# nirschl-lab/stain2stain

Measured on AMD Instinct MI355X. Metric: paired 256x256 stain tiles/sec (full CFM optimisation step), higher is better.
Workload: dtype bf16

## Files before the change

stain2stain_amd/csrc/conv3x3_wgrad_mfma.hip:

```cpp
#include "common.h"
#include <stdlib.h>
#include <type_traits>

struct WgradArgs {
  const void* dy;
  const void* x0;
  const void* x1;
  float* part;
  int lddy, Cout, ld0, c0, ld1, c1;
  int B, H, W, tilesY, tilesX, ntiles, S;
  int lgc;
  int lgh, lgw;
  int xcd;
};

namespace {

template <typename T> struct WPiece;
template <> struct WPiece<bf16_t> {
  bf16x8 v;
  __device__ __forceinline__ void zero() {
#pragma unroll
    for (int i = 0; i < 8; ++i) v[i] = (bf16_t)0.0f;
  }
  __device__ __forceinline__ void load(const bf16_t* p) { v = *reinterpret_cast<const bf16x8*>(p); }
  __device__ __forceinline__ void to_lds(char* hi, int, int off) const { *reinterpret_cast<bf16x8*>(hi + off) = v; }
};
template <> struct WPiece<float> {
  f32x4 a, b;
  __device__ __forceinline__ void zero() {
#pragma unroll
    for (int i = 0; i < 4; ++i) { a[i] = 0.f; b[i] = 0.f; }
  }
  __device__ __forceinline__ void load(const float* p) {
    a = *reinterpret_cast<const f32x4*>(p);
    b = *reinterpret_cast<const f32x4*>(p + 4);
  }
  __device__ __forceinline__ void to_lds(char* hi, int img_stride, int off) const {
    bf16x8 h, m, l;
#pragma unroll
    for (int i = 0; i < 8; ++i) {
      const float x = i < 4 ? a[i] : b[i - 4];
      h[i] = (bf16_t)x;
      const float r1 = x - (float)h[i];
      m[i] = (bf16_t)r1;
      l[i] = (bf16_t)(r1 - (float)m[i]);
    }
    *reinterpret_cast<bf16x8*>(hi + off) = h;
    *reinterpret_cast<bf16x8*>(hi + img_stride + off) = m;
    *reinterpret_cast<bf16x8*>(hi + 2 * img_stride + off) = l;
  }
};

typedef __attribute__((address_space(3))) s16x4 lds_s16x4;

__device__ __forceinline__ bf16x8 tr_frag(const char* p_rows0, int row_stride4) {
  s16x4 lo = __builtin_amdgcn_ds_read_tr16_b64_v4i16((lds_s16x4*)(p_rows0));
  s16x4 hi = __builtin_amdgcn_ds_read_tr16_b64_v4i16((lds_s16x4*)(p_rows0 + row_stride4));
  bf16x4 l4 = __builtin_bit_cast(bf16x4, lo), h4 = __builtin_bit_cast(bf16x4, hi);
  bf16x8 r;
#pragma unroll
  for (int i = 0; i < 4; ++i) { r[i] = l4[i]; r[4 + i] = h4[i]; }
  return r;
}

template <typename T, int TH, int TW>
__global__ __launch_bounds__(256, (std::is_same<T, float>::value ? 1 : 2)) void conv3x3_wgrad_kernel(WgradArgs a) {
  constexpr bool SPLIT = std::is_same<T, float>::value;
  constexpr int NIMG = SPLIT ? 3 : 1;
  constexpr int NPX = TH * TW;
  constexpr int HW_ = TW + 2, HALO = (TH + 2) * HW_;
  constexpr int DY_BYTES = 2 * NPX * 64;
  constexpr int X_BYTES = 2 * HALO * 64;
  constexpr int DY_PIECES = NPX * 8, DY_IT = (DY_PIECES + 255) / 256;
  constexpr int X_PIECES = HALO * 8, X_IT = (X_PIECES + 255) / 256;
  constexpr int KSTEPS = NPX / 16;
  static_assert(TW % 16 == 0, "a k-step is 16 consecutive pixels of one tile row");

  extern __shared__ __attribute__((aligned(16))) char smem[];
  char* const ldsDY = smem;
  char* const ldsX = smem + NIMG * DY_BYTES;

  const T* __restrict__ dy = static_cast<const T*>(a.dy);
  const T* __restrict__ x0 = static_cast<const T*>(a.x0);
  const T* __restrict__ x1 = static_cast<const T*>(a.x1);

  const int tid = threadIdx.x, lane = tid & 63, wave = tid >> 6;
  const int wco = wave >> 1, wci = wave & 1;
  const int ci0 = blockIdx.x * 64, co0 = blockIdx.y * 64;
  const int cin = a.c0 + a.c1;

  const int g = lane >> 4, q = (lane & 15) >> 2, p = lane & 3;
  const int frag_off = ((g >> 1) * 8 + q) * 64 + ((g & 1) * 16 + p * 4) * 2;

  f32x16 acc[9];
#pragma unroll
  for (int t = 0; t < 9; ++t)
#pragma unroll
    for (int j = 0; j < 16; ++j) acc[t][j] = 0.f;

  WPiece<T> dreg[DY_IT];
  WPiece<T> xreg[X_IT];

  auto load_tile = [&](int tile) {
    int bt = tile;
    const int tx = bt % a.tilesX; bt /= a.tilesX;
    const int ty = bt % a.tilesY;
    const int img = bt / a.tilesY;
    const int y0 = ty * TH, xs = tx * TW;
#pragma unroll
    for (int i = 0; i < DY_IT; ++i) {
      const int idx = tid + i * 256;
      const int px = idx >> 3, pc = idx & 7;
      const int py = px / TW, pxx = px - py * TW;
      const int gy = y0 + py, gx = xs + pxx, co = co0 + pc * 8;
      dreg[i].zero();
      if (idx < DY_PIECES && gy < a.H && gx < a.W && co < a.Cout)
        dreg[i].load(dy + ((long)(img * a.H + gy) * a.W + gx) * a.lddy + co);
    }
#pragma unroll
    for (int i = 0; i < X_IT; ++i) {
      const int idx = tid + i * 256;
      const int px = idx >> 3, pc = idx & 7;
      const int hy = px / HW_, hx = px - hy * HW_;
      const int gy = y0 - 1 + hy, gx = xs - 1 + hx, ci = ci0 + pc * 8;
      xreg[i].zero();
      if (idx < X_PIECES && gy >= 0 && gy < a.H && gx >= 0 && gx < a.W) {
        const long pix = (long)(img * a.H + gy) * a.W + gx;
        if (ci < a.c0) xreg[i].load(x0 + pix * a.ld0 + ci);
        else if (ci < cin) xreg[i].load(x1 + pix * a.ld1 + (ci - a.c0));
      }
    }
  };
  auto store_tile = [&]() {
#pragma unroll
    for (int i = 0; i < DY_IT; ++i) {
      const int idx = tid + i * 256;
      const int px = idx >> 3, pc = idx & 7;
      if (idx < DY_PIECES)
        dreg[i].to_lds(ldsDY, DY_BYTES, (pc >> 2) * (NPX * 64) + px * 64 + (pc & 3) * 16);
    }
#pragma unroll
    for (int i = 0; i < X_IT; ++i) {
      const int idx = tid + i * 256;
      const int px = idx >> 3, pc = idx & 7;
      if (idx < X_PIECES)
        xreg[i].to_lds(ldsX, X_BYTES, (pc >> 2) * (HALO * 64) + px * 64 + (pc & 3) * 16);
    }
  };

  const char* const Ahi = ldsDY + wco * (NPX * 64) + frag_off;
  const char* const Bhi = ldsX + wci * (HALO * 64) + frag_off;

  int tile = blockIdx.z;
  if (tile < a.ntiles) load_tile(tile);
  for (; tile < a.ntiles; tile += a.S) {
    __syncthreads();
    store_tile();
    __syncthreads();
    if (tile + a.S < a.ntiles) load_tile(tile + a.S);
#pragma unroll
    for (int ks = 0; ks < KSTEPS; ++ks) {
      const int m0 = ks * 16;
      const int py = m0 / TW, px = m0 - py * TW;
      const bf16x8 af = tr_frag(Ahi + m0 * 64, 4 * 64);
      bf16x8 am, al;
// ... 3 lines not shown
      }
#pragma unroll
      for (int tap = 0; tap < 9; ++tap) {
        const int hoff = ((py + tap / 3) * HW_ + px + tap % 3) * 64;
        const bf16x8 bfr = tr_frag(Bhi + hoff, 4 * 64);
        if constexpr (SPLIT) {
          const bf16x8 bm = tr_frag(Bhi + X_BYTES + hoff, 4 * 64);
          const bf16x8 bl = tr_frag(Bhi + 2 * X_BYTES + hoff, 4 * 64);
          acc[tap] = __builtin_amdgcn_mfma_f32_32x32x16_bf16(am, bm, acc[tap], 0, 0, 0);
          acc[tap] = __builtin_amdgcn_mfma_f32_32x32x16_bf16(al, bfr, acc[tap], 0, 0, 0);
          acc[tap] = __builtin_amdgcn_mfma_f32_32x32x16_bf16(af, bl, acc[tap], 0, 0, 0);
          acc[tap] = __builtin_amdgcn_mfma_f32_32x32x16_bf16(am, bfr, acc[tap], 0, 0, 0);
          acc[tap] = __builtin_amdgcn_mfma_f32_32x32x16_bf16(af, bm, acc[tap], 0, 0, 0);
        }
        acc[tap] = __builtin_amdgcn_mfma_f32_32x32x16_bf16(af, bfr, acc[tap], 0, 0, 0);
      }
    }
  }

  const int r = lane & 31, h = lane >> 5;
  const int ci = ci0 + wci * 32 + r;
#pragma unroll
  for (int tap = 0; tap < 9; ++tap) {
#pragma unroll
    for (int j = 0; j < 16; ++j) {
      const int co = co0 + wco * 32 + (j & 3) + 8 * (j >> 2) + 4 * h;
      if (co < a.Cout && ci < cin)
        a.part[(((long)blockIdx.z * 9 + tap) * a.Cout + co) * cin + ci] = acc[tap][j];
    }
  }
}

__device__ __attribute__((aligned(64))) char g_wgrad_zero_page[64];
typedef __attribute__((address_space(3))) void lds_void_t;
typedef __attribute__((address_space(1))) const void gbl_void_t;

__device__ __forceinline__ void dma16_asm(const void* gsrc, unsigned lds_dst) {
  unsigned keep;
  asm volatile("s_mov_b32 %0, m0\n\ts_mov_b32 m0, %2\n\ts_nop 0\n\tglobal_load_lds_dwordx4 %1, off\n\ts_mov_b32 m0, %0"
               : "=&s"(keep) : "v"(gsrc), "s"(lds_dst) : "memory");
}

template <int TH, int TW>
__global__ __launch_bounds__(256, 2) void conv3x3_wgrad_dma_kernel(WgradArgs a) {
  using T = bf16_t;
  constexpr int NW = 4, NT = 9;
  constexpr int NPX = TH * TW;
  constexpr int HW_ = TW + 2, HR = TH + 2, HALO = HR * HW_;
  constexpr int XROWS = (HALO + 31) / 32 * 32;
  constexpr int DY_BYTES = 2 * NPX * 64, X_BYTES = 2 * XROWS * 64;
  constexpr int DYGRP = 2 * NPX / 16, XGRP = 2 * XROWS / 16;
  constexpr int DYG = DYGRP / NW;
  constexpr int XG = XGRP / NW;
  constexpr int BUF = DY_BYTES + X_BYTES;
  constexpr int KSTEPS = NPX / 16;
  static_assert(DYGRP % 4 == 0 && XGRP % 4 == 0, "DMA groups split evenly over 4 waves");

  extern __shared__ __attribute__((aligned(16))) char smem[];
  const T* __restrict__ dy = static_cast<const T*>(a.dy);
  const T* __restrict__ x0 = static_cast<const T*>(a.x0);
  const T* __restrict__ x1 = static_cast<const T*>(a.x1);

  const int tid = threadIdx.x, lane = tid & 63;
  const int wave = __builtin_amdgcn_readfirstlane(tid >> 6);
  const int wco = (wave & 3) >> 1, wci = wave & 1;
  unsigned bx = blockIdx.x, by = blockIdx.y, bz = blockIdx.z;
  if (a.xcd) {
    const unsigned L = bx + gridDim.x * (by + gridDim.y * bz), per = gridDim.x * gridDim.y * gridDim.z / 8;
    unsigned Lq = (L & 7) * per + (L >> 3);
    bx = Lq % gridDim.x; Lq /= gridDim.x;
    by = Lq % gridDim.y; bz = Lq / gridDim.y;
  }
  const int ci0 = bx * 64, co0 = by * 64;
  const int cin = a.c0 + a.c1;
  const int drow = lane >> 2, dslot = lane & 3;
  const int zsplit = (int)bz;

  const int g = lane >> 4, q = (lane & 15) >> 2, p = lane & 3;
  const int frag_off = ((g >> 1) * 8 + q) * 64 + ((g & 1) * 16 + p * 4) * 2;

  f32x16 acc[NT];
#pragma unroll
  for (int t = 0; t < NT; ++t)
#pragma unroll
    for (int j = 0; j < 16; ++j) acc[t][j] = 0.f;

  int dy_off[DYG], dy_py[DYG], dy_px[DYG];
  bool dy_ok[DYG];
#pragma unroll
  for (int j = 0; j < DYG; ++j) {
    const int grp = wave + NW * j;
    const int half = grp / (NPX / 16), px = (grp % (NPX / 16)) * 16 + drow;
    const int co = co0 + half * 32 + dslot * 8;
    dy_py[j] = px / TW; dy_px[j] = px - dy_py[j] * TW;
    dy_ok[j] = co < a.Cout;
    dy_off[j] = (dy_py[j] * a.W + dy_px[j]) * a.lddy + co;
  }
  const T* x_ptr[XG];
  int x_off[XG], x_ld[XG], x_hy[XG], x_hx[XG];
#pragma unroll
  for (int j = 0; j < XG; ++j) {
    const int grp = wave + NW * j;
    const int half = grp / (XROWS / 16), px = (grp % (XROWS / 16)) * 16 + drow;
    const int ci = ci0 + half * 32 + dslot * 8;
    x_hy[j] = px / HW_; x_hx[j] = px - x_hy[j] * HW_;
    x_ptr[j] = nullptr; x_ld[j] = 0;
    if (px < HALO) {
      if (ci < a.c0) { x_ptr[j] = x0 + ci; x_ld[j] = a.ld0; }
      else if (ci < cin) { x_ptr[j] = x1 + (ci - a.c0); x_ld[j] = a.ld1; }
    }
    x_off[j] = ((x_hy[j] - 1) * a.W + (x_hx[j] - 1)) * x_ld[j];
  }

  auto dma_tile = [&](int tile, int buf) {
    int bt = tile;
    const int tx = bt % a.tilesX; bt /= a.tilesX;
    const int ty = bt % a.tilesY;
    const int img = bt / a.tilesY;
    const int y0 = ty * TH, xs = tx * TW;
    const long pixbase = (long)(img * a.H + y0) * a.W + xs;
    const bool interior = y0 >= 1 && y0 + TH + 1 <= a.H && xs >= 1 && xs + TW + 1 <= a.W;
    const unsigned base = (unsigned)(uintptr_t)(__attribute__((address_space(3))) char*)smem + buf * BUF;
    if (interior) {
#pragma unroll
      for (int j = 0; j < DYG; ++j) {
        const void* src = dy_ok[j] ? (const void*)(dy + pixbase * a.lddy + dy_off[j]) : (const void*)g_wgrad_zero_page;
        dma16_asm(src, __builtin_amdgcn_readfirstlane(base + (wave + NW * j) * 1024));
      }
#pragma unroll
      for (int j = 0; j < XG; ++j) {
        const void* src = x_ptr[j] ? (const void*)(x_ptr[j] + pixbase * x_ld[j] + x_off[j]) : (const void*)g_wgrad_zero_page;
        dma16_asm(src, __builtin_amdgcn_readfirstlane(base + DY_BYTES + (wave + NW * j) * 1024));
      }
    } else {
#pragma unroll
      for (int j = 0; j < DYG; ++j) {
        const int gy = y0 + dy_py[j], gx = xs + dy_px[j];
        const void* src = g_wgrad_zero_page;
        if (gy < a.H && gx < a.W && dy_ok[j]) src = dy + pixbase * a.lddy + dy_off[j];
        dma16_asm(src, __builtin_amdgcn_readfirstlane(base + (wave + NW * j) * 1024));
      }
#pragma unroll
      for (int j = 0; j < XG; ++j) {
        const int gy = y0 - 1 + x_hy[j], gx = xs - 1 + x_hx[j];
        const void* src = g_wgrad_zero_page;
        if (x_ptr[j] && gy >= 0 && gy < a.H && gx >= 0 && gx < a.W) src = x_ptr[j] + pixbase * x_ld[j] + x_off[j];
        dma16_asm(src, __builtin_amdgcn_readfirstlane(base + DY_BYTES + (wave + NW * j) * 1024));
      }
    }
  };

  int tile = zsplit;
  int buf = 0;
  if (tile < a.ntiles) dma_tile(tile, 0);
  asm volatile("s_waitcnt vmcnt(0)" ::: "memory");
  __builtin_amdgcn_s_barrier();
  for (; tile < a.ntiles; tile += a.S) {
    if (tile + a.S < a.ntiles) dma_tile(tile + a.S, buf ^ 1);
    const char* const Ahi = smem + buf * BUF + wco * (NPX * 64) + frag_off;
    const char* const Bhi = smem + buf * BUF + DY_BYTES + wci * (XROWS * 64) + frag_off;
#pragma unroll
    for (int ks = 0; ks < KSTEPS; ++ks) {
      const int m0 = ks * 16;
      const int py = m0 / TW, px = m0 - py * TW;
      const bf16x8 af = tr_frag(Ahi + m0 * 64, 4 * 64);
#pragma unroll
      for (int t = 0; t < NT; ++t) {
        const int hoff = ((py + t / 3) * HW_ + px + t % 3) * 64;
        const bf16x8 bfr = tr_frag(Bhi + hoff, 4 * 64);
        acc[t] = __builtin_amdgcn_mfma_f32_32x32x16_bf16(af, bfr, acc[t], 0, 0, 0);
      }
    }
    __builtin_amdgcn_sched_barrier(0);
    asm volatile("s_waitcnt vmcnt(0)" ::: "memory");
    __builtin_amdgcn_s_barrier();
    buf ^= 1;
  }

  const int r = lane & 31, h = lane >> 5;
  const int ci = ci0 + wci * 32 + r;
#pragma unroll
  for (int t = 0; t < NT; ++t) {
#pragma unroll
    for (int j = 0; j < 16; ++j) {
      const int co = co0 + wco * 32 + (j & 3) + 8 * (j >> 2) + 4 * h;
      if (co < a.Cout && ci < cin)
        a.part[(((long)zsplit * 9 + t) * a.Cout + co) * cin + ci] = acc[t][j];
    }
  }
}

template <int ZG>
__global__ __launch_bounds__(64 * ZG) void wgrad_reduce_kernel(const float* __restrict__ part, float* __restrict__ grad, int S, int Cout,
                                    int Cin, int accumulate) {
  __shared__ float tile[ZG][9][65];
  const long n = (long)Cout * Cin;
  const int il = threadIdx.x & 63, zg = threadIdx.x >> 6;
  const long i = (long)blockIdx.x * 64 + il;
  float s[9];
#pragma unroll
  for (int t = 0; t < 9; ++t) s[t] = 0.f;
  if (i < n) {
    for (int z = zg; z < S; z += ZG)
#pragma unroll
      for (int t = 0; t < 9; ++t) s[t] += part[((long)z * 9 + t) * n + i];
  }
#pragma unroll
  for (int t = 0; t < 9; ++t) tile[zg][t][il] = s[t];
  __syncthreads();
  const long base = (long)blockIdx.x * 64 * 9;
  for (int k = threadIdx.x; k < 576; k += 64 * ZG) {
    const long o = base + k;
    if (o < n * 9) {
      const int t = k % 9, j = k / 9;
      float v = 0.f;
#pragma unroll
      for (int g = 0; g < ZG; g += 4) v += (tile[g][t][j] + tile[g + 1][t][j]) + (tile[g + 2][t][j] + tile[g + 3][t][j]);
      grad[o] = accumulate ? grad[o] + v : v;
    }
  }
}

template <typename T, int TH, int TW>
int launch_wgrad(WgradArgs& a, hipStream_t s) {
  constexpr int NIMG = std::is_same<T, float>::value ? 3 : 1;
  constexpr int lds = NIMG * (2 * TH * TW * 64 + 2 * (TH + 2) * (TW + 2) * 64);
  a.tilesY = cdiv(a.H, TH);
  a.tilesX = cdiv(a.W, TW);
  a.ntiles = a.B * a.tilesY * a.tilesX;
  if (a.S > a.ntiles) return S2S_ERR_SHAPE;
  auto kern = conv3x3_wgrad_kernel<T, TH, TW>;
  static unsigned long long attr_devs = 0;
  if (int rc = s2s_allow_dyn_lds(reinterpret_cast<const void*>(kern), lds, &attr_devs)) return rc;
  dim3 grid(cdiv(a.c0 + a.c1, 64), cdiv(a.Cout, 64), a.S);
  hipLaunchKernelGGL(kern, grid, dim3(256), lds, s, a);
  S2S_LAUNCH_CHECK();
  return S2S_OK;
}

template <int TH, int TW>
int launch_wgrad_dma(WgradArgs& a, hipStream_t s) {
  constexpr int XROWS = ((TH + 2) * (TW + 2) + 31) / 32 * 32;
  constexpr int lds = 2 * (2 * TH * TW * 64 + 2 * XROWS * 64);
  a.tilesY = cdiv(a.H, TH);
  a.tilesX = cdiv(a.W, TW);
  a.ntiles = a.B * a.tilesY * a.tilesX;
  if (a.S > a.ntiles) return S2S_ERR_SHAPE;
  auto kern = conv3x3_wgrad_dma_kernel<TH, TW>;
  static unsigned long long attr_devs = 0;
  if (int rc = s2s_allow_dyn_lds(reinterpret_cast<const void*>(kern), lds, &attr_devs)) return rc;
  dim3 grid(cdiv(a.c0 + a.c1, 64), cdiv(a.Cout, 64), a.S);
  static const int xcd_aware = [] { const char* e = getenv("S2S_WGRAD_XCD"); return e ? atoi(e) : 1; }();
  a.xcd = xcd_aware && ((long)grid.x * grid.y * grid.z) % 8 == 0;
  hipLaunchKernelGGL(kern, grid, dim3(256), lds, s, a);
  S2S_LAUNCH_CHECK();
  return S2S_OK;
}

template <int TH, int TW, bool S2D = false>
__global__ __launch_bounds__(256, 2) void conv2x2_wgrad_dma_kernel(WgradArgs a) {
  using T = bf16_t;
  constexpr int NT = 4;
  constexpr int NPX = TH * TW;
  constexpr int HW_ = TW + 1, HR = TH + 1, HALO = HR * HW_;
  constexpr int XROWS = (HALO + 31) / 32 * 32;
  constexpr int DY_BYTES = 2 * NPX * 64, X_BYTES = 2 * XROWS * 64;
  constexpr int DYG = 2 * NPX / 16 / 4;
  constexpr int XG = 2 * XROWS / 16 / 4;
  constexpr int BUF = DY_BYTES + X_BYTES;
  constexpr int KSTEPS = NPX / 16;
  static_assert((2 * NPX / 16) % 4 == 0 && (2 * XROWS / 16) % 4 == 0, "DMA groups split evenly over 4 waves");

  extern __shared__ __attribute__((aligned(16))) char smem[];
  const T* __restrict__ dy = static_cast<const T*>(a.dy);
  const T* __restrict__ x0 = static_cast<const T*>(a.x0);

  const int tid = threadIdx.x, lane = tid & 63;
  const int wave = __builtin_amdgcn_readfirstlane(tid >> 6);
  const int wco = wave >> 1, wci = wave & 1;
  const int ci0 = blockIdx.x * 64, co0 = blockIdx.y * 64;
  const int cin = a.c0;
  const int Hi = a.H + 1, Wi = a.W + 1;
  const int drow = lane >> 2, dslot = lane & 3;
  const int zsplit = (int)blockIdx.z;

  const int g = lane >> 4, q = (lane & 15) >> 2, p = lane & 3;
  const int frag_off = ((g >> 1) * 8 + q) * 64 + ((g & 1) * 16 + p * 4) * 2;

  f32x16 acc[NT];
#pragma unroll
  for (int t = 0; t < NT; ++t)
#pragma unroll
    for (int j = 0; j < 16; ++j) acc[t][j] = 0.f;

  int dy_off[DYG], dy_py[DYG], dy_px[DYG];
  bool dy_ok[DYG];
#pragma unroll
  for (int j = 0; j < DYG; ++j) {
    const int grp = wave + 4 * j;
    const int half = grp / (NPX / 16), px = (grp % (NPX / 16)) * 16 + drow;
    const int co = co0 + half * 32 + dslot * 8;
    dy_py[j] = px / TW; dy_px[j] = px - dy_py[j] * TW;
    dy_ok[j] = co < a.Cout;
    dy_off[j] = (dy_py[j] * a.W + dy_px[j]) * a.lddy + co;
  }
  const T* x_ptr[XG];
  int x_off[XG], x_hy[XG], x_hx[XG];
#pragma unroll
  for (int j = 0; j < XG; ++j) {
    const int grp = wave + 4 * j;
    const int half = grp / (XROWS / 16), px = (grp % (XROWS / 16)) * 16 + drow;
    const int ci = ci0 + half * 32 + dslot * 8;
    x_hy[j] = px / HW_; x_hx[j] = px - x_hy[j] * HW_;
    if (S2D) {
      const int rs = ci >> a.lgc;
      x_ptr[j] = (px < HALO && ci < cin) ? x0 + (ci & ((1 << a.lgc) - 1)) : nullptr;
      x_hy[j] = 2 * x_hy[j] + (rs >> 1) - 1;
      x_hx[j] = 2 * x_hx[j] + (rs & 1) - 1;
      x_off[j] = 0;
    } else {
      x_ptr[j] = (px < HALO && ci < cin) ? x0 + ci : nullptr;
      x_off[j] = (x_hy[j] * Wi + x_hx[j]) * a.ld0;
    }
  }

  auto dma_tile = [&](int tile, int buf) {
    int bt = tile;
    const int tx = bt % a.tilesX; bt /= a.tilesX;
    const int ty = bt % a.tilesY;
    const int img = bt / a.tilesY;
    const int y0 = ty * TH, xs = tx * TW;
    const long pixbase = (long)(img * a.H + y0) * a.W + xs;
    const long xbase = (long)(img * Hi + y0) * Wi + xs;
    const bool interior = !S2D && y0 + TH <= a.H && xs + TW <= a.W;
    const unsigned base = (unsigned)(uintptr_t)(__attribute__((address_space(3))) char*)smem + buf * BUF;
    if (interior) {
#pragma unroll
      for (int j = 0; j < DYG; ++j) {
        const void* src = dy_ok[j] ? (const void*)(dy + pixbase * a.lddy + dy_off[j]) : (const void*)g_wgrad_zero_page;
        dma16_asm(src, __builtin_amdgcn_readfirstlane(base + (wave + 4 * j) * 1024));
      }
#pragma unroll
      for (int j = 0; j < XG; ++j) {
        const void* src = x_ptr[j] ? (const void*)(x_ptr[j] + xbase * a.ld0 + x_off[j]) : (const void*)g_wgrad_zero_page;
        dma16_asm(src, __builtin_amdgcn_readfirstlane(base + DY_BYTES + (wave + 4 * j) * 1024));
      }
    } else {
#pragma unroll
      for (int j = 0; j < DYG; ++j) {
        const int gy = y0 + dy_py[j], gx = xs + dy_px[j];
        const void* src = g_wgrad_zero_page;
        if (gy < a.H && gx < a.W && dy_ok[j]) src = dy + pixbase * a.lddy + dy_off[j];
        dma16_asm(src, __builtin_amdgcn_readfirstlane(base + (wave + 4 * j) * 1024));
      }
#pragma unroll
      for (int j = 0; j < XG; ++j) {
        const void* src = g_wgrad_zero_page;
        if (S2D) {
          const int py = 2 * y0 + x_hy[j], px = 2 * xs + x_hx[j];
          if (x_ptr[j] && (unsigned)py < (unsigned)(2 * a.H) && (unsigned)px < (unsigned)(2 * a.W))
            src = x_ptr[j] + ((long)(img * 2 * a.H + py) * (2 * a.W) + px) * a.ld0;
        } else {
          const int gy = y0 + x_hy[j], gx = xs + x_hx[j];
          if (x_ptr[j] && gy < Hi && gx < Wi) src = x_ptr[j] + xbase * a.ld0 + x_off[j];
        }
        dma16_asm(src, __builtin_amdgcn_readfirstlane(base + DY_BYTES + (wave + 4 * j) * 1024));
      }
    }
  };

  int tile = zsplit;
  int buf = 0;
  if (tile < a.ntiles) dma_tile(tile, 0);
  asm volatile("s_waitcnt vmcnt(0)" ::: "memory");
  __builtin_amdgcn_s_barrier();
  for (; tile < a.ntiles; tile += a.S) {
    if (tile + a.S < a.ntiles) dma_tile(tile + a.S, buf ^ 1);
    const char* const Ahi = smem + buf * BUF + wco * (NPX * 64) + frag_off;
    const char* const Bhi = smem + buf * BUF + DY_BYTES + wci * (XROWS * 64) + frag_off;
#pragma unroll
    for (int ks = 0; ks < KSTEPS; ++ks) {
      const int m0 = ks * 16;
      const int py = m0 / TW, px = m0 - py * TW;
      const bf16x8 af = tr_frag(Ahi + m0 * 64, 4 * 64);
#pragma unroll
      for (int t = 0; t < NT; ++t) {
        const int hoff = ((py + t / 2) * HW_ + px + t % 2) * 64;
        const bf16x8 bfr = tr_frag(Bhi + hoff, 4 * 64);
        acc[t] = __builtin_amdgcn_mfma_f32_32x32x16_bf16(af, bfr, acc[t], 0, 0, 0);
      }
    }
    __builtin_amdgcn_sched_barrier(0);
    asm volatile("s_waitcnt vmcnt(0)" ::: "memory");
    __builtin_amdgcn_s_barrier();
    buf ^= 1;
  }

  const int r = lane & 31, h = lane >> 5;
  const int ci = ci0 + wci * 32 + r;
#pragma unroll
  for (int t = 0; t < NT; ++t) {
#pragma unroll
    for (int j = 0; j < 16; ++j) {
      const int co = co0 + wco * 32 + (j & 3) + 8 * (j >> 2) + 4 * h;
      if (co < a.Cout && ci < cin)
        a.part[(((long)zsplit * NT + t) * a.Cout + co) * cin + ci] = acc[t][j];
    }
  }
}

__global__ __launch_bounds__(256, 1) void conv2x2_wgrad_flat_kernel(WgradArgs a) {
// ... 397 lines not shown
  };
  const char* const Ahi = ldsDY + wco * (NPX * 64) + frag_off;
  const char* const Bhi = ldsX + wci * (HALO * 64) + frag_off;

  int tile = zsplit;
  if (tile < a.ntiles) load_tile(tile);
  for (; tile < a.ntiles; tile += a.S) {
    __syncthreads();
    store_tile();
    __syncthreads();
    if (tile + a.S < a.ntiles) load_tile(tile + a.S);
#pragma unroll
    for (int ks = 0; ks < KSTEPS; ++ks) {
      const int m0 = ks * 16;
      const int py = m0 / TW, px = m0 - py * TW;
      const bf16x8 af = tr_frag(Ahi + m0 * 64, 4 * 64);
      bf16x8 am, al;
      if constexpr (SPLIT) {
        am = tr_frag(Ahi + DY_BYTES + m0 * 64, 4 * 64);
        al = tr_frag(Ahi + 2 * DY_BYTES + m0 * 64, 4 * 64);
      }
#pragma unroll
      for (int t = 0; t < NT; ++t) {
        const int hoff = (py * HW_ + px + t) * 64;
        const bf16x8 bfr = tr_frag(Bhi + hoff, 4 * 64);
        if constexpr (SPLIT) {
          const bf16x8 bm = tr_frag(Bhi + X_BYTES + hoff, 4 * 64);
          const bf16x8 bl = tr_frag(Bhi + 2 * X_BYTES + hoff, 4 * 64);
          acc[t] = __builtin_amdgcn_mfma_f32_32x32x16_bf16(am, bm, acc[t], 0, 0, 0);
          acc[t] = __builtin_amdgcn_mfma_f32_32x32x16_bf16(al, bfr, acc[t], 0, 0, 0);
          acc[t] = __builtin_amdgcn_mfma_f32_32x32x16_bf16(af, bl, acc[t], 0, 0, 0);
          acc[t] = __builtin_amdgcn_mfma_f32_32x32x16_bf16(am, bfr, acc[t], 0, 0, 0);
          acc[t] = __builtin_amdgcn_mfma_f32_32x32x16_bf16(af, bm, acc[t], 0, 0, 0);
        }
        acc[t] = __builtin_amdgcn_mfma_f32_32x32x16_bf16(af, bfr, acc[t], 0, 0, 0);
      }
    }
  }
  const int r = lane & 31, h = lane >> 5;
  const int ci = ci0 + wci * 32 + r;
#pragma unroll
  for (int t = 0; t < NT; ++t) {
    const int tap = kh * KS + t;
#pragma unroll
    for (int j = 0; j < 16; ++j) {
      const int co = co0 + wco * 32 + (j & 3) + 8 * (j >> 2) + 4 * h;
      if (co < a.Cout && ci < cin) a.part[(((long)zsplit * (KS * KS) + tap) * a.Cout + co) * cin + ci] = acc[t][j];
    }
  }
}

template <int ZG>
__global__ __launch_bounds__(256 * ZG) void wgrad_fold4x4_kernel(const float* __restrict__ part, float* __restrict__ grad, int S,
                                                                 int Cout, int C, int mode, int accumulate) {
  __shared__ float tile[ZG][16][65];
  const int o = blockIdx.y, c0 = blockIdx.x * 64;
  const int cl = threadIdx.x & 63, grp = (threadIdx.x >> 6) & 3, zg = threadIdx.x >> 8;
  const long slab = 16L * Cout * C;
#pragma unroll
  for (int i = 0; i < 4; ++i) {
    const int t16 = grp + 4 * i, kh = t16 >> 2, kw = t16 & 3;
    long src;
    if (mode == 1) src = ((long)((kh >> 1) * 2 + (kw >> 1)) * Cout + o) * (4L * C) + ((kh & 1) * 2 + (kw & 1)) * C + c0 + cl;
    else src = ((long)t16 * Cout + o) * C + c0 + cl;
    float acc[8];
#pragma unroll
    for (int k = 0; k < 8; ++k) acc[k] = 0.f;
    if (c0 + cl < C) {
      int z = zg;
      for (; z + 7 * ZG < S; z += 8 * ZG) {
#pragma unroll
        for (int k = 0; k < 8; ++k) acc[k] += part[(long)(z + k * ZG) * slab + src];
      }
      for (; z < S; z += ZG) acc[0] += part[(long)z * slab + src];
    }
    tile[zg][t16][cl] = ((acc[0] + acc[1]) + (acc[2] + acc[3])) + ((acc[4] + acc[5]) + (acc[6] + acc[7]));
  }
  __syncthreads();
  const long base = ((long)o * C + c0) * 16;
  for (int k = threadIdx.x; k < 1024; k += 256 * ZG) {
    const int c = k >> 4, t16 = k & 15;
    if (c0 + c < C) {
      float v = 0.f;
#pragma unroll
      for (int g = 0; g < ZG; ++g) v += tile[g][t16][c];
      grad[base + k] = accumulate ? grad[base + k] + v : v;
    }
  }
}

__global__ __launch_bounds__(256) void split_sum_kernel(const float* __restrict__ part, float* __restrict__ out, int S, long n,
                                                        int accumulate) {
  const long i = (long)blockIdx.x * 256 + threadIdx.x;
  if (i >= n) return;
  float s0 = 0.f, s1 = 0.f;
  int z = 0;
  for (; z + 1 < S; z += 2) { s0 += part[(long)z * n + i]; s1 += part[(long)(z + 1) * n + i]; }
  if (z < S) s0 += part[(long)z * n + i];
  const float v = s0 + s1;
  out[i] = accumulate ? out[i] + v : v;
}

int p2p_wgrad_target() {
  static const int t = [] { const char* e = getenv("S2S_P2P_WGRAD_BLOCKS"); const int v = e ? atoi(e) : 0; return v > 0 ? v : 256; }();
  return t;
}

int conv2x2_wgrad_splits(int B, int H, int W, int Cin, int Cout) {
  const int nt = B * cdiv(H, 8) * cdiv(W, 16);
  const int mn = cdiv(Cin, 64) * cdiv(Cout, 64);
  int s = p2p_wgrad_target() / mn;
  if (s > 256) s = 256;
  if (s > nt) s = nt;
  if (s < 1) s = 1;
  return s;
}

int wgrad_ntiles(int B, int H, int W) { return B * cdiv(H, 8) * cdiv(W, 16); }

}

extern "C" int s2s_conv3x3_wgrad_splits(int dtype, int B, int H, int W, int Cin, int Cout) {
  if (B <= 0 || H <= 0 || W <= 0 || Cin <= 0 || Cout <= 0) return S2S_ERR_SHAPE;
  const int nt = wgrad_ntiles(B, H, W);
  const int mn = cdiv(Cin, 64) * cdiv(Cout, 64);
  static const int target_env = [] { const char* e = getenv("S2S_WGRAD_BLOCKS"); return e ? atoi(e) : 0; }();
  const int target = target_env ? target_env : 256;
  const int cap = mn == 1 ? 512 : 320;
  int s = target / mn;
  if (target_env == 0 && s >= 1 && (long)s * mn < (long)target * 7 / 8 && (long)(s + 1) * mn <= 2L * target) s += 1;
  if (s > cap) s = cap;
  if (s > nt) s = nt;
  if (s < 1) s = 1;
  return s;
}

extern "C" int s2s_conv3x3_wgrad_phase(int dtype, const void* dy, int lddy, int Cout, const void* x0, int ld0, int c0,
                                       const void* x1, int ld1, int c1, float* part, float* grad_oihw,
                                       int accumulate, int B, int H, int W, int phases, void* stream) {
  if (!dy || !x0 || !part || !grad_oihw) return S2S_ERR_NULL;
  if (phases < 1 || phases > 3) return S2S_ERR_SHAPE;
  if (B <= 0 || H <= 0 || W <= 0 || Cout <= 0 || c0 <= 0 || c1 < 0) return S2S_ERR_SHAPE;
  if ((Cout % 8) || (c0 % 8) || (c1 % 8) || (lddy % 8) || (ld0 % 8) || (ld1 % 8) || (c1 > 0 && !x1)) return S2S_ERR_SHAPE;
  if (((uintptr_t)dy & 15) || ((uintptr_t)x0 & 15) || ((uintptr_t)x1 & 15)) return S2S_ERR_ALIGN;
  WgradArgs a{};
  a.dy = dy; a.x0 = x0; a.x1 = x1; a.part = part;
  a.lddy = lddy; a.Cout = Cout; a.ld0 = ld0; a.c0 = c0; a.ld1 = ld1; a.c1 = c1;
  a.B = B; a.H = H; a.W = W; a.lgc = 0; a.lgh = a.lgw = 0;
  a.S = s2s_conv3x3_wgrad_splits(dtype, B, H, W, c0 + c1, Cout);
  hipStream_t s = static_cast<hipStream_t>(stream);
  int rc = S2S_OK;
  if (dtype != S2S_BF16 && dtype != S2S_F32) return S2S_ERR_DTYPE;
  if (!(phases & 1)) { if (a.S > wgrad_ntiles(B, H, W)) return S2S_ERR_SHAPE; }
  else if (dtype == S2S_BF16) rc = launch_wgrad_dma<8, 16>(a, s);
  else rc = launch_wgrad<float, 8, 16>(a, s);
  if (rc != S2S_OK || !(phases & 2)) return rc;
  const long n = (long)Cout * (c0 + c1);
  if (n <= 32768 && a.S >= 32)
    hipLaunchKernelGGL(wgrad_reduce_kernel<16>, dim3((unsigned)((n + 63) / 64)), dim3(1024), 0, s, part, grad_oihw,
                       a.S, Cout, c0 + c1, accumulate);
  else
    hipLaunchKernelGGL(wgrad_reduce_kernel<4>, dim3((unsigned)((n + 63) / 64)), dim3(256), 0, s, part, grad_oihw,
                       a.S, Cout, c0 + c1, accumulate);
  S2S_LAUNCH_CHECK();
  return S2S_OK;
}

extern "C" int s2s_conv3x3_wgrad_nhwc(int dtype, const void* dy, int lddy, int Cout, const void* x0, int ld0, int c0,
                                      const void* x1, int ld1, int c1, float* part, float* grad_oihw,
                                      int accumulate, int B, int H, int W, void* stream) {
  return s2s_conv3x3_wgrad_phase(dtype, dy, lddy, Cout, x0, ld0, c0, x1, ld1, c1, part, grad_oihw, accumulate, B, H, W, 3,
                                 stream);
}

extern "C" int s2s_conv2x2_wgrad_splits(int B, int H, int W, int Cin, int Cout) {
  if (B <= 0 || H <= 0 || W <= 0 || Cin <= 0 || Cout <= 0) return S2S_ERR_SHAPE;
  return conv2x2_wgrad_splits(B, H, W, Cin, Cout);
}

extern "C" int s2s_conv2x2_wgrad_nhwc(int dtype, const void* dy, int lddy, int Cout, const void* x, int ldx, int cin,
                                      float* part, float* grad2, int accumulate, int B, int H, int W, void* stream) {
  if (!dy || !x || !part || !grad2) return S2S_ERR_NULL;
  if (dtype != S2S_BF16) return S2S_ERR_DTYPE;
  if (B <= 0 || H <= 0 || W <= 0 || Cout <= 0 || cin <= 0) return S2S_ERR_SHAPE;
  if ((Cout % 8) || (cin % 8) || (lddy % 8) || (ldx % 8)) return S2S_ERR_SHAPE;
  if (((uintptr_t)dy & 15) || ((uintptr_t)x & 15)) return S2S_ERR_ALIGN;
  if ((long)B * (H + 1) * (W + 1) >= (1L << 31)) return S2S_ERR_SHAPE;
  WgradArgs a{};
  a.dy = dy; a.x0 = x; a.x1 = nullptr; a.part = part;
  a.lddy = lddy; a.Cout = Cout; a.ld0 = ldx; a.c0 = cin; a.ld1 = 8; a.c1 = 0;
  a.B = B; a.H = H; a.W = W; a.lgc = 0; a.lgh = a.lgw = 0;
  a.S = conv2x2_wgrad_splits(B, H, W, cin, Cout);
  a.tilesY = cdiv(H, 8); a.tilesX = cdiv(W, 16);
  a.ntiles = B * a.tilesY * a.tilesX;
  hipStream_t s = static_cast<hipStream_t>(stream);
  constexpr int TH = 8, TW = 16;
  constexpr int XROWS = ((TH + 1) * (TW + 1) + 31) / 32 * 32;
  constexpr int lds = 2 * (2 * TH * TW * 64 + 2 * XROWS * 64);
  auto kern = conv2x2_wgrad_dma_kernel<TH, TW>;
  static unsigned long long attr_devs = 0;
  if (int rc = s2s_allow_dyn_lds(reinterpret_cast<const void*>(kern), lds, &attr_devs)) return rc;
  dim3 grid(cdiv(cin, 64), cdiv(Cout, 64), a.S);
  hipLaunchKernelGGL(kern, grid, dim3(256), lds, s, a);
  const long n = 4L * Cout * cin;
  hipLaunchKernelGGL(split_sum_kernel, dim3((unsigned)((n + 255) / 256)), dim3(256), 0, s, part, grad2, a.S, n,
                     accumulate);
  S2S_LAUNCH_CHECK();
  return S2S_OK;
}

extern "C" int s2s_conv4x4s1_wgrad_splits(int B, int H, int W, int Cin, int Cout) {
  if (B <= 0 || H <= 0 || W <= 0 || Cin <= 0 || Cout <= 0) return S2S_ERR_SHAPE;
  const int nt = B * cdiv(H, 8) * cdiv(W, 16);
  const int mn = cdiv(Cin, 64) * cdiv(Cout, 64) * 4;
  static const int t1 = [] { const char* e = getenv("S2S_P2P_WGRAD_S1_BLOCKS"); const int v = e ? atoi(e) : 0; return v > 0 ? v : 384; }();
  int s = t1 / mn;
  if (s > 128) s = 128;
  if (s > nt) s = nt;
  if (s < 1) s = 1;
  return s;
}

extern "C" int s2s_conv4x4s1_wgrad_nhwc(int dtype, const void* dy, int lddy, int Cout, const void* x, int ldx, int cin,
                                        float* part, float* grad16, int accumulate, int B, int H, int W,
                                        void* stream) {
  if (!dy || !x || !part || !grad16) return S2S_ERR_NULL;
  if (dtype != S2S_BF16) return S2S_ERR_DTYPE;
  if (B <= 0 || H <= 0 || W <= 0 || Cout <= 0 || cin <= 0) return S2S_ERR_SHAPE;
  if ((Cout % 8) || (cin % 8) || (lddy % 8) || (ldx % 8)) return S2S_ERR_SHAPE;
  if (((uintptr_t)dy & 15) || ((uintptr_t)x & 15)) return S2S_ERR_ALIGN;
  if ((long)B * (H + 1) * (W + 1) >= (1L << 31)) return S2S_ERR_SHAPE;
  WgradArgs a{};
  a.dy = dy; a.x0 = x; a.x1 = nullptr; a.part = part;
  a.lddy = lddy; a.Cout = Cout; a.ld0 = ldx; a.c0 = cin; a.ld1 = 8; a.c1 = 0;
  a.B = B; a.H = H; a.W = W; a.lgc = 0; a.lgh = a.lgw = 0;
  a.S = s2s_conv4x4s1_wgrad_splits(B, H, W, cin, Cout);
  a.tilesY = cdiv(H, 8); a.tilesX = cdiv(W, 16);
  a.ntiles = B * a.tilesY * a.tilesX;
  hipStream_t s = static_cast<hipStream_t>(stream);
  constexpr int TH = 8, TW = 16, KS = 4;
  constexpr int XROWS = (TH * (TW + KS - 1) + 31) / 32 * 32;
  constexpr int lds = 2 * (2 * TH * TW * 64 + 2 * XROWS * 64);
  auto kern = convkxk_wgrad_rows_kernel<TH, TW, KS, 1>;
  static unsigned long long attr_devs = 0;
  if (int rc = s2s_allow_dyn_lds(reinterpret_cast<const void*>(kern), lds, &attr_devs)) return rc;
  dim3 grid(cdiv(cin, 64), cdiv(Cout, 64), a.S * KS);
  hipLaunchKernelGGL(kern, grid, dim3(256), lds, s, a);
  const long n = 16L * Cout * cin;
  hipLaunchKernelGGL(split_sum_kernel, dim3((unsigned)((n + 255) / 256)), dim3(256), 0, s, part, grad16, a.S, n,
                     accumulate);
  S2S_LAUNCH_CHECK();
  return S2S_OK;
}

extern "C" int s2s_convkxk_wgrad_splits(int dtype, int B, int H, int W, int Cin, int Cout, int ks) {
  if (B <= 0 || H <= 0 || W <= 0 || Cin <= 0 || Cout <= 0 || (ks != 2 && ks != 4)) return S2S_ERR_SHAPE;
  if (dtype != S2S_BF16 && dtype != S2S_F32) return S2S_ERR_DTYPE;
  if (dtype == S2S_BF16 && ks == 2) return conv2x2_wgrad_splits(B, H, W, Cin, Cout);
  if (dtype == S2S_BF16) return s2s_conv4x4s1_wgrad_splits(B, H, W, Cin, Cout);
  const int nt = B * cdiv(H, 8) * cdiv(W, 16);
  const int mn = cdiv(Cin, 64) * cdiv(Cout, 64) * ks;
  int s = 512 / mn;
  if (s > 128) s = 128;
  if (s > nt) s = nt;
  if (s < 1) s = 1;
  return s;
}

template <typename T, int KS, int PAD>
static int launch_wgrad_rs(WgradArgs& a, hipStream_t s) {
  constexpr int TH = 8, TW = 16;
  constexpr int NIMG = std::is_same<T, float>::value ? 3 : 1;
  constexpr int lds = NIMG * (2 * TH * TW * 64 + 2 * TH * (TW + KS - 1) * 64);
  static_assert(lds <= 160 * 1024, "LDS budget");
  auto kern = convkxk_wgrad_rs_kernel<T, TH, TW, KS, PAD>;
  static unsigned long long attr_devs = 0;
  if (int rc = s2s_allow_dyn_lds(reinterpret_cast<const void*>(kern), lds, &attr_devs)) return rc;
  dim3 grid(cdiv(a.c0, 64), cdiv(a.Cout, 64), a.S * KS);
  hipLaunchKernelGGL(kern, grid, dim3(256), lds, s, a);
  return S2S_OK;
}

extern "C" int s2s_convkxk_wgrad_nhwc(int dtype, const void* dy, int lddy, int Cout, const void* x, int ldx, int cin,
                                      float* part, float* grad, int layout, int accumulate, int B, int H, int W, int ks,
                                      int x_plain, void* stream) {
  if (!dy || !x || !part || !grad) return S2S_ERR_NULL;
  if (dtype != S2S_BF16 && dtype != S2S_F32) return S2S_ERR_DTYPE;
  if (B <= 0 || H <= 0 || W <= 0 || Cout <= 0 || cin <= 0 || (ks != 2 && ks != 4)) return S2S_ERR_SHAPE;
  if ((Cout % 8) || (cin % 8) || (lddy % 8) || (ldx % 8) || (layout != 0 && layout != 1)) return S2S_ERR_SHAPE;
  if (ks == 2 && layout == 1 && (cin % 32)) return S2S_ERR_SHAPE;
  if (x_plain && (dtype != S2S_BF16 || ks != 2 || (cin % 32) || ((cin / 4) & (cin / 4 - 1)) || ldx < cin / 4)) return S2S_ERR_SHAPE;
  if (x_plain && (H >= 16384 || W >= 16384)) return S2S_ERR_SHAPE;
  if (((uintptr_t)dy & 15) || ((uintptr_t)x & 15)) return S2S_ERR_ALIGN;
  if ((long)B * (H + 1) * (W + 1) >= (1L << 31)) return S2S_ERR_SHAPE;
  WgradArgs a{};
  a.dy = dy; a.x0 = x; a.x1 = nullptr; a.part = part;
  a.lddy = lddy; a.Cout = Cout; a.ld0 = ldx; a.c0 = cin; a.ld1 = 8; a.c1 = 0;
  a.B = B; a.H = H; a.W = W; a.lgc = 0; a.lgh = a.lgw = 0;
  a.S = s2s_convkxk_wgrad_splits(dtype, B, H, W, cin, Cout, ks);
  a.tilesY = cdiv(H, 8); a.tilesX = cdiv(W, 16);
  a.ntiles = B * a.tilesY * a.tilesX;
  hipStream_t s = static_cast<hipStream_t>(stream);
  constexpr int TH = 8, TW = 16;
  int rc = S2S_OK;
  if (dtype == S2S_F32) {
    rc = ks == 2 ? launch_wgrad_rs<float, 2, 0>(a, s) : launch_wgrad_rs<float, 4, 1>(a, s);
  } else if (ks == 2) {
// ... 61 lines not shown
```

Baseline: 2244.

## Add 3-stage ring-buffered wgrad kernel with buffer-resource DMA and partial vmcnt waits

Result: no change. 2257 (median of 6 runs) (+0.6%).

```diff
diff --git a/stain2stain_amd/csrc/conv3x3_wgrad_mfma.hip b/stain2stain_amd/csrc/conv3x3_wgrad_mfma.hip
--- a/stain2stain_amd/csrc/conv3x3_wgrad_mfma.hip
+++ b/stain2stain_amd/csrc/conv3x3_wgrad_mfma.hip
@@ -1,6 +1,12 @@
 #include "common.h"
 #include <stdlib.h>
 #include <type_traits>
+
+#ifdef S2S_ABLATE
+#define S2S_ABL(cond) (cond)
+#else
+#define S2S_ABL(cond) false
+#endif
 
 struct WgradArgs {
   const void* dy;
@@ -12,6 +18,7 @@
   int lgc;
   int lgh, lgw;
   int xcd;
+  int dbg;
 };
 
 namespace {
@@ -321,13 +328,14 @@
 
   int tile = zsplit;
   int buf = 0;
-  if (tile < a.ntiles) dma_tile(tile, 0);
+  if (tile < a.ntiles && !S2S_ABL(a.dbg & 1)) dma_tile(tile, 0);
   asm volatile("s_waitcnt vmcnt(0)" ::: "memory");
   __builtin_amdgcn_s_barrier();
   for (; tile < a.ntiles; tile += a.S) {
-    if (tile + a.S < a.ntiles) dma_tile(tile + a.S, buf ^ 1);
+    if (tile + a.S < a.ntiles && !S2S_ABL(a.dbg & 1)) dma_tile(tile + a.S, buf ^ 1);
     const char* const Ahi = smem + buf * BUF + wco * (NPX * 64) + frag_off;
     const char* const Bhi = smem + buf * BUF + DY_BYTES + wci * (XROWS * 64) + frag_off;
+    if (!S2S_ABL(a.dbg & 2))
 #pragma unroll
     for (int ks = 0; ks < KSTEPS; ++ks) {
       const int m0 = ks * 16;
@@ -345,6 +353,180 @@
     __builtin_amdgcn_s_barrier();
     buf ^= 1;
   }
+  if (S2S_ABL(a.dbg & 4)) return;
+
+  const int r = lane & 31, h = lane >> 5;
+  const int ci = ci0 + wci * 32 + r;
+#pragma unroll
+  for (int t = 0; t < NT; ++t) {
+#pragma unroll
+    for (int j = 0; j < 16; ++j) {
+      const int co = co0 + wco * 32 + (j & 3) + 8 * (j >> 2) + 4 * h;
+      if (co < a.Cout && ci < cin)
+        a.part[(((long)zsplit * 9 + t) * a.Cout + co) * cin + ci] = acc[t][j];
+    }
+  }
+}
+
+typedef __attribute__((ext_vector_type(4))) unsigned u32x4;
+
+__device__ __forceinline__ u32x4 wgrad_rsrc(const void* base, long nbytes) {
+  const unsigned long b = (unsigned long)base;
+  u32x4 r;
+  r[0] = (unsigned)b;
+  r[1] = (unsigned)(b >> 32) & 0xffffu;
+  r[2] = nbytes <= 0 ? 0u : nbytes >= 0x7fffffffL ? 0x7fffffffu : (unsigned)nbytes;
+  r[3] = 0x00020000u;
+  return r;
+}
+
+__device__ __forceinline__ void bdma16_asm(u32x4 rsrc, unsigned voff, unsigned lds_dst) {
+  unsigned keep;
+  asm volatile("s_nop 4\n\ts_mov_b32 %0, m0\n\ts_mov_b32 m0, %3\n\ts_nop 0\n\tbuffer_load_dwordx4 %1, %2, 0 offen lds\n\t"
+               "s_mov_b32 m0, %0"
+               : "=&s"(keep) : "v"(voff), "s"(rsrc), "s"(lds_dst) : "memory");
+}
+
+template <int N>
+__device__ __forceinline__ void wgrad_wait_vm() {
+  asm volatile("s_waitcnt vmcnt(%0)" ::"n"(N) : "memory");
+}
+
+template <int TH, int TW, int NS>
+__global__ __launch_bounds__(256, 2) void conv3x3_wgrad_ring_kernel(WgradArgs a) {
+  using T = bf16_t;
+  constexpr int NW = 4, NT = 9;
+  constexpr int NPX = TH * TW;
+  constexpr int HW_ = TW + 2, HR = TH + 2, HALO = HR * HW_;
+  constexpr int XROWS = (HALO + 31) / 32 * 32;
+  constexpr int DY_BYTES = 2 * NPX * 64, X_BYTES = 2 * XROWS * 64;
+  constexpr int DYGRP = 2 * NPX / 16, XGRP = 2 * XROWS / 16;
+  constexpr int DYG = DYGRP / NW, XG = XGRP / NW;
+  constexpr int NDMA = DYG + XG;
+  constexpr int BUF = DY_BYTES + X_BYTES;
+  constexpr int KSTEPS = NPX / 16;
+  constexpr unsigned OOB = 0xffffff00u;
+  static_assert((NPX / 16) % NW == 0 && (XROWS / 16) % NW == 0, "a wave's DMA groups of one half are whole j steps");
+  static_assert(NS >= 2 && NS <= 4 && (NS - 2) * NDMA <= 63, "vmcnt is a 6-bit counter");
+
+  extern __shared__ __attribute__((aligned(16))) char smem[];
+  const T* __restrict__ dy = static_cast<const T*>(a.dy);
+
+  const int tid = threadIdx.x, lane = tid & 63;
+  const int wave = __builtin_amdgcn_readfirstlane(tid >> 6);
+  const int wco = (wave & 3) >> 1, wci = wave & 1;
+  unsigned bx = blockIdx.x, by = blockIdx.y, bz = blockIdx.z;
+  if (a.xcd) {
+    const unsigned L = bx + gridDim.x * (by + gridDim.y * bz), per = gridDim.x * gridDim.y * gridDim.z / 8;
+    unsigned Lq = (L & 7) * per + (L >> 3);
+    bx = Lq % gridDim.x; Lq /= gridDim.x;
+    by = Lq % gridDim.y; bz = Lq / gridDim.y;
+  }
+  const int ci0 = bx * 64, co0 = by * 64;
+  const int cin = a.c0 + a.c1;
+  const int drow = lane >> 2, dslot = lane & 3;
+  const int zsplit = (int)bz;
+  const long npix = (long)a.B * a.H * a.W;
+
+  const int g = lane >> 4, q = (lane & 15) >> 2, p = lane & 3;
+  const int frag_off = ((g >> 1) * 8 + q) * 64 + ((g & 1) * 16 + p * 4) * 2;
+
+  f32x16 acc[NT];
+#pragma unroll
+  for (int t = 0; t < NT; ++t)
+#pragma unroll
+    for (int j = 0; j < 16; ++j) acc[t][j] = 0.f;
+
+  const T* xsrc[2];
+  int xch[2], xleft[2], xld[2];
+#pragma unroll
+  for (int h = 0; h < 2; ++h) {
+    const int c = ci0 + 32 * h;
+    const bool first = c < a.c0;
+    xsrc[h] = first ? static_cast<const T*>(a.x0) : (a.c1 ? static_cast<const T*>(a.x1) : static_cast<const T*>(a.x0));
+    xch[h] = first ? c : c - a.c0;
+    xleft[h] = first ? a.c0 - c : (a.c1 ? a.c1 - (c - a.c0) : 0);
+    xld[h] = first ? a.ld0 : a.ld1;
+  }
+
+  unsigned dy_off[DYG], x_off[XG];
+  int dy_py[DYG], dy_px[DYG], x_hy[XG], x_hx[XG];
+#pragma unroll
+  for (int j = 0; j < DYG; ++j) {
+    const int grp = wave + NW * j, half = j / (DYG / 2);
+    const int px = (grp % (NPX / 16)) * 16 + drow;
+    const int co = co0 + half * 32 + dslot * 8;
+    dy_py[j] = px / TW; dy_px[j] = px - dy_py[j] * TW;
+    dy_off[j] = co < a.Cout ? (unsigned)(((dy_py[j] * a.W + dy_px[j]) * a.lddy + co) * 2) : OOB;
+  }
+#pragma unroll
+  for (int j = 0; j < XG; ++j) {
+    const int grp = wave + NW * j, half = j / (XG / 2);
+    const int px = (grp % (XROWS / 16)) * 16 + drow;
+    x_hy[j] = px / HW_; x_hx[j] = px - x_hy[j] * HW_;
+    const bool ok = px < HALO && dslot * 8 < xleft[half];
+    x_off[j] = ok ? (unsigned)(((x_hy[j] * a.W + x_hx[j]) * xld[half] + dslot * 8) * 2) : OOB;
+  }
+
+  auto dma_tile = [&](int tile, int st) {
+    if (S2S_ABL(a.dbg & 1)) return;
+    int bt = tile;
+    const int tx = bt % a.tilesX; bt /= a.tilesX;
+    const int ty = bt % a.tilesY;
+    const int img = bt / a.tilesY;
+    const int y0 = ty * TH, xs = tx * TW;
+    const long pix = (long)(img * a.H + y0) * a.W + xs;
+    const long pixh = pix - a.W - 1;
+    const unsigned base = (unsigned)(uintptr_t)(__attribute__((address_space(3))) char*)smem + st * BUF;
+    const u32x4 rdy = wgrad_rsrc(dy + pix * a.lddy, ((npix - 1 - pix) * a.lddy + a.Cout) * 2);
+    const int ylim = a.H - y0, xlim = a.W - xs;
+#pragma unroll
+    for (int j = 0; j < DYG; ++j) {
+      const unsigned off = (dy_py[j] < ylim && dy_px[j] < xlim) ? dy_off[j] : OOB;
+      bdma16_asm(rdy, off, __builtin_amdgcn_readfirstlane(base + (wave + NW * j) * 1024));
+    }
+#pragma unroll
+    for (int h = 0; h < 2; ++h) {
+      const u32x4 rx = wgrad_rsrc(xsrc[h] + pixh * xld[h] + xch[h], ((npix - 1 - pixh) * xld[h] + xleft[h]) * 2);
+#pragma unroll
+      for (int j = h * (XG / 2); j < (h + 1) * (XG / 2); ++j) {
+        const bool in = (unsigned)(y0 - 1 + x_hy[j]) < (unsigned)a.H && (unsigned)(xs - 1 + x_hx[j]) < (unsigned)a.W;
+        bdma16_asm(rx, in ? x_off[j] : OOB, __builtin_amdgcn_readfirstlane(base + DY_BYTES + (wave + NW * j) * 1024));
+      }
+    }
+  };
+
+  const int n = zsplit < a.ntiles ? (a.ntiles - 1 - zsplit) / a.S + 1 : 0;
+#pragma unroll
+  for (int i = 0; i < NS - 1; ++i)
+    if (i < n) dma_tile(zsplit + i * a.S, i);
+  int st = 0;
+  for (int i = 0; i < n; ++i) {
+    const int younger = n - 1 - i;
+    if constexpr (NS >= 4) { if (younger >= 2) wgrad_wait_vm<2 * NDMA>(); else if (younger == 1) wgrad_wait_vm<NDMA>(); else wgrad_wait_vm<0>(); }
+    else if constexpr (NS == 3) { if (younger >= 1) wgrad_wait_vm<NDMA>(); else wgrad_wait_vm<0>(); }
+    else wgrad_wait_vm<0>();
+    __builtin_amdgcn_s_barrier();
+    if (i + NS - 1 < n) dma_tile(zsplit + (i + NS - 1) * a.S, st == 0 ? NS - 1 : st - 1);
+    const char* const Ahi = smem + st * BUF + wco * (NPX * 64) + frag_off;
+    const char* const Bhi = smem + st * BUF + DY_BYTES + wci * (XROWS * 64) + frag_off;
+    if (!S2S_ABL(a.dbg & 2))
+#pragma unroll
+    for (int ks = 0; ks < KSTEPS; ++ks) {
+      const int m0 = ks * 16;
+      const int py = m0 / TW, px = m0 - py * TW;
+      const bf16x8 af = tr_frag(Ahi + m0 * 64, 4 * 64);
+#pragma unroll
+      for (int t = 0; t < NT; ++t) {
+        const int hoff = ((py + t / 3) * HW_ + px + t % 3) * 64;
+        const bf16x8 bfr = tr_frag(Bhi + hoff, 4 * 64);
+        acc[t] = __builtin_amdgcn_mfma_f32_32x32x16_bf16(af, bfr, acc[t], 0, 0, 0);
+      }
+    }
+    __builtin_amdgcn_sched_barrier(0);
+    st = st == NS - 1 ? 0 : st + 1;
+  }
+  if (S2S_ABL(a.dbg & 4)) return;
 
   const int r = lane & 31, h = lane >> 5;
   const int ci = ci0 + wci * 32 + r;
@@ -426,6 +608,47 @@
   return S2S_OK;
 }
 
+bool wgrad_ring_fits(const WgradArgs& a, int TH) {
+  const long ld = a.lddy > a.ld0 ? (a.lddy > a.ld1 ? a.lddy : a.ld1) : (a.ld0 > a.ld1 ? a.ld0 : a.ld1);
+  return a.c0 % 32 == 0 && (long)(TH + 2) * a.W * ld * 2 < 0x7fff0000L;
+}
+
+template <int TH, int TW, int NS>
+int launch_wgrad_ring(WgradArgs& a, hipStream_t s) {
+  constexpr int XROWS = ((TH + 2) * (TW + 2) + 31) / 32 * 32;
+  constexpr int lds = NS * (2 * TH * TW * 64 + 2 * XROWS * 64);
+  a.tilesY = cdiv(a.H, TH);
+  a.tilesX = cdiv(a.W, TW);
+  a.ntiles = a.B * a.tilesY * a.tilesX;
+  if (a.S > a.ntiles) return S2S_ERR_SHAPE;
+  auto kern = conv3x3_wgrad_ring_kernel<TH, TW, NS>;
+  static unsigned long long attr_devs = 0;
+  if (int rc = s2s_allow_dyn_lds(reinterpret_cast<const void*>(kern), lds, &attr_devs)) return rc;
+  dim3 grid(cdiv(a.c0 + a.c1, 64), cdiv(a.Cout, 64), a.S);
+  static const int xcd_aware = [] { const char* e = getenv("S2S_WGRAD_XCD"); return e ? atoi(e) : 1; }();
+  a.xcd = xcd_aware && ((long)grid.x * grid.y * grid.z) % 8 == 0;
+  hipLaunchKernelGGL(kern, grid, dim3(256), lds, s, a);
+  S2S_LAUNCH_CHECK();
+  return S2S_OK;
+}
+
+int launch_wgrad_bf16(WgradArgs& a, hipStream_t s) {
+#ifdef S2S_ABLATE
+  static const int dbg = [] { const char* e = getenv("S2S_WGRAD_DBG"); return e ? atoi(e) : 0; }();
+  static const int ring = [] { const char* e = getenv("S2S_WGRAD_RING"); return e ? atoi(e) : 3; }();
+  a.dbg = dbg;
+  if (ring && wgrad_ring_fits(a, 8)) {
+    if (ring == 2) return launch_wgrad_ring<8, 16, 2>(a, s);
+    if (ring == 4) return launch_wgrad_ring<8, 16, 4>(a, s);
+    return launch_wgrad_ring<8, 16, 3>(a, s);
+  }
+  return launch_wgrad_dma<8, 16>(a, s);
+#else
+  if (wgrad_ring_fits(a, 8)) return launch_wgrad_ring<8, 16, 3>(a, s);
+  return launch_wgrad_dma<8, 16>(a, s);
+#endif
+}
+
 template <int TH, int TW, bool S2D = false>
 __global__ __launch_bounds__(256, 2) void conv2x2_wgrad_dma_kernel(WgradArgs a) {
   using T = bf16_t;
@@ -1129,7 +1352,7 @@
   int rc = S2S_OK;
   if (dtype != S2S_BF16 && dtype != S2S_F32) return S2S_ERR_DTYPE;
   if (!(phases & 1)) { if (a.S > wgrad_ntiles(B, H, W)) return S2S_ERR_SHAPE; }
-  else if (dtype == S2S_BF16) rc = launch_wgrad_dma<8, 16>(a, s);
+  else if (dtype == S2S_BF16) rc = launch_wgrad_bf16(a, s);
   else rc = launch_wgrad<float, 8, 16>(a, s);
   if (rc != S2S_OK || !(phases & 2)) return rc;
   const long n = (long)Cout * (c0 + c1);
```
